# G-U-N/consolver

Measured on AMD Instinct MI355X. Metric: images/sec at 8-step ConsistencySolver 512x512 (final latents; SD1.5 UNet fp16 + PPOScheduler, CFG 3), higher is better.
Workload: dtype f16

## Files before the change

### consolver_amd/csrc/igemm.hip

```cpp
#include "ops.h"
#include <stdlib.h>
#include <type_traits>


namespace {

constexpr int BM = 128;
constexpr int BK = 64;

__device__ __attribute__((aligned(256))) unsigned g_zero_page[64];

struct IgemmParams {
    const f16* a0; const f16* a1; int c0, c1;
    int Hi, Wi, Ho, Wo, HoWo;
    int stride, upsample;
    int pad_lo;
    int M, N, KT, cpt;
    int Ktot;
    const f16* w; const f16* bias; const f16* temb; int temb_stride; const f16* res; f16* out;
    const f16* res_lo; f16* out_lo;
    const f16* a0_lo; const f16* a1_lo; int KTh;
    float* row_stats;
    const float* ln_stats; int ln_groups; float ln_inv_c, ln_eps; const float* ln_s; const float* ln_b;
    int tiles_n, nblk;
// ... 1305 lines not shown
    asm volatile("s_waitcnt vmcnt(0)" ::: "memory");
    __builtin_amdgcn_s_barrier();
    if (KT > 1) static_for<4>([&](auto nc) { piece(nc, 1, 1); });
    lds_read<0>(fw[0], SW[0][0]); lds_read<0>(fa[0][0], SA[0][0]); lds_read<2048>(fa[0][1], SA[0][0]);
    lds_read<2048>(fw[1], SW[0][0]); lds_read<2 * 2048>(fa[0][2], SA[0][0]); lds_read<3 * 2048>(fa[0][3], SA[0][0]);
    lds_read<2 * 2048>(fw[2], SW[0][0]); lds_read<3 * 2048>(fw[3], SW[0][0]);

    int kt = 0;
    auto step = [&](auto b_tag) {
        constexpr int B = decltype(b_tag)::value, BO = B ^ 1;
        static_for<NQ>([&](auto qc) {
            constexpr int q = decltype(qc)::value, ks = q / NT, i = q - ks * NT;
            if constexpr (q == QB) {
                asm volatile("s_waitcnt vmcnt(0) lgkmcnt(0)" ::: "memory");
                __builtin_amdgcn_s_barrier();
            }
            {
                constexpr int r = q + LA;
                if constexpr (r < NT) lds_read<r * 2048>(fw[r % RS], SW[B][0]);
                else if constexpr (r < NQ) lds_read<(r - NT) * 2048>(fw[r % RS], SW[B][1]);
                else lds_read<(r - NQ) * 2048>(fw[r % RS], SW[BO][0]);
            }
            if constexpr (q < MT) lds_read<q * 2048>(fa[1][q], SA[B][1]);
            if constexpr (q == QB || q == QB + 1) {
                constexpr int j0 = (q - QB) * 2;
                lds_read<j0 * 2048>(fa[0][j0], SA[BO][0]); lds_read<(j0 + 1) * 2048>(fa[0][j0 + 1], SA[BO][0]);
            }
            asm volatile("s_waitcnt lgkmcnt(%0)" :: "n"(lw_wait_count(q, NQ, LA, MT, QB)));
            __builtin_amdgcn_sched_barrier(0);
#pragma unroll
            for (int j = 0; j < MT; ++j) mfma_inplace(acc[i][j], fw[q % RS], fa[ks][j]);
            __builtin_amdgcn_sched_barrier(0);
            if constexpr (q < 5) { if (kt + 1 < KT) piece(std::integral_constant<int, 4 + q>{}, kt + 1, BO); }
            if constexpr (q >= QB) { if (kt + 2 < KT) piece(std::integral_constant<int, q - QB>{}, kt + 2, B); }
            __builtin_amdgcn_sched_barrier(0);
        });
    };
    for (;;) {
        step(std::integral_constant<int, 0>{}); if (++kt == KT) break;
        step(std::integral_constant<int, 1>{}); if (++kt == KT) break;
    }
    asm volatile("s_waitcnt vmcnt(0) lgkmcnt(0)\n s_nop 7\n s_nop 7" ::: "memory");
#pragma unroll
    for (int i = 0; i < NT; ++i)
#pragma unroll
        for (int j = 0; j < MT; ++j) asm volatile("" : "+v"(acc[i][j]));
    __builtin_amdgcn_s_barrier();
    char* const ln_tab = LNM == 1 ? lnx + BMX * 8 + wn * (2 * (BNX / 2) * 4) : lnx + wn * (BNX / 2) * 2;
    const char* const ln_rows = LNM == 1 ? lnx + wm * 64 * 8 : nullptr;
    if constexpr (GEGLU) igemm_epilogue<GEGLU, NT, MT, NT, LinearRows, 1, LNM, true>(p, acc, LinearRows{m_blk + wm * 64, p.M}, n_blk + wn * (BNX / 2), lane, smem + w * 11264, ln_tab, ln_rows);
    else igemm_epilogue<GEGLU, NT, MT, NT, LinearRows, 2, LNM, true, EPI>(p, acc, LinearRows{m_blk + wm * 64, p.M}, n_blk + wn * (BNX / 2), lane, smem + w * 11264, ln_tab, ln_rows);
}

__global__ __launch_bounds__(256) void row_stats_kernel(const f16* __restrict__ x, const f16* __restrict__ x_lo, int M, int C, float* __restrict__ stats, int lo8) {
    const int lane = threadIdx.x & 63, row = blockIdx.x * 4 + (threadIdx.x >> 6);
    if (row >= M) return;
    float s1 = 0.f, s2 = 0.f;
    for (int c = lane * 8; c < C; c += 512) {
        const f16x8 t = *reinterpret_cast<const f16x8*>(x + (size_t)row * C + c);
        float fv[8];
#pragma unroll
        for (int k = 0; k < 8; ++k) fv[k] = (float)t[k];
        if (x_lo && lo8) lo8_decode_add(fv, *reinterpret_cast<const u32x2_t*>(reinterpret_cast<const unsigned char*>(x_lo) + (size_t)row * C + c));
        else if (x_lo) {
            const f16x8 t2 = *reinterpret_cast<const f16x8*>(x_lo + (size_t)row * C + c);
#pragma unroll
            for (int k = 0; k < 8; ++k) fv[k] += (float)t2[k];
        }
#pragma unroll
        for (int k = 0; k < 8; ++k) { const float f = fv[k]; s1 += f; s2 = __builtin_fmaf(f, f, s2); }
    }
    s1 = wave_sum(s1); s2 = wave_sum(s2);
    if (lane == 0) { stats[2 * (size_t)row] = s1; stats[2 * (size_t)row + 1] = s2; }
}

__device__ __forceinline__ f16x8 splitk_reduce_item(const IgemmParams& p, const float* __restrict__ partial, int splits, int m, int n) {
    float v[8] = {0, 0, 0, 0, 0, 0, 0, 0};
    for (int s = 0; s < splits; ++s) {
        const float* src = partial + ((size_t)s * p.M + m) * p.N + n;
        const f32x4 a = *reinterpret_cast<const f32x4*>(src), b = *reinterpret_cast<const f32x4*>(src + 4);
#pragma unroll
        for (int k = 0; k < 4; ++k) { v[k] += a[k]; v[4 + k] += b[k]; }
    }
    if (p.ln_stats) {
        float s1 = 0.f, s2 = 0.f;
        const float* st = p.ln_stats + (size_t)m * p.ln_groups * 2;
        ln_row_moments(st, p.ln_groups, s1, s2);
        const float mean = s1 * p.ln_inv_c, rstd = __builtin_amdgcn_rsqf(fmaxf(__builtin_fmaf(-mean, mean, s2 * p.ln_inv_c), 0.f) + p.ln_eps), mr = mean * rstd;
#pragma unroll
        for (int k = 0; k < 8; ++k) v[k] = __builtin_fmaf(v[k], rstd, __builtin_fmaf(-mr, p.ln_s[n + k], p.ln_b[n + k]));
    } else if (p.bias) { const f16x8 t = *reinterpret_cast<const f16x8*>(p.bias + n);
#pragma unroll
        for (int k = 0; k < 8; ++k) v[k] += (float)t[k]; }
    if (p.temb) { const f16x8 t = *reinterpret_cast<const f16x8*>(p.temb + (size_t)(m / p.HoWo) * p.temb_stride + n);
#pragma unroll
        for (int k = 0; k < 8; ++k) v[k] += (float)t[k]; }
    if (p.res) { const f16x8 t = *reinterpret_cast<const f16x8*>(p.res + (size_t)m * p.N + n);
#pragma unroll
        for (int k = 0; k < 8; ++k) v[k] += (float)t[k]; }
    if (p.res && p.res_lo) {
        if (p.lo8) lo8_decode_add(v, *reinterpret_cast<const u32x2_t*>(reinterpret_cast<const unsigned char*>(p.res_lo) + (size_t)m * p.N + n));
        else { const f16x8 t = *reinterpret_cast<const f16x8*>(p.res_lo + (size_t)m * p.N + n);
#pragma unroll
            for (int k = 0; k < 8; ++k) v[k] += (float)t[k]; }
    }
    f16x8 o;
// ... 368 lines not shown
        configured = true;
    }
    hipLaunchKernelGGL(kfn, dim3(p.nblk, splits), dim3(256), lds, s, p);
    CS_CHECK_LAUNCH();
    if (splits > 1) return launch_splitk_reduce(p, (const float*)p.partial, splits, s);
    return CS_OK;
}

}

constexpr size_t LN_LDS_W8 = 256 * 8 + 2 * 2 * 160 * 4, LN_LDS_LW = 256 * 8 + 2 * 160 * 4;

static int choose_xcd_grid(int tiles_m, int tiles_n, double a_bytes, double w_bytes) {
    if (!tune().xcd_grid) return 0;
    int best = 0; double best_cost = 0.85 * (a_bytes + 8.0 * w_bytes);
    for (int pn = 2; pn <= 8; pn *= 2) {
        const int px = 8 / pn;
        if (tiles_n % pn || tiles_m % px) continue;
        const double cost = pn * a_bytes + px * w_bytes;
        if (cost < best_cost) { best_cost = cost; best = pn; }
    }
    return best;
}

double igemm_flops(const IgemmArgs& a) {
    const double M = (double)a.B * a.Ho * a.Wo;
    return 2.0 * M * a.N * (double)a.taps * (a.c0 + a.c1);
}

template <bool UP, int BN, int KH, int SCHED>
static int launch_halo_sched(const HaloParams& h, dim3 grid, size_t lds, hipStream_t s) {
    static bool configured = false;
    if (!configured) {
        constexpr size_t max_lds = 2 * (HALO_ROWS_MAX * 128) + 3 * (160 * 128);
        CS_CHECK_HIP(hipFuncSetAttribute(reinterpret_cast<const void*>(conv3_halo_kernel<UP, BN, KH, SCHED>), hipFuncAttributeMaxDynamicSharedMemorySize, (int)max_lds));
        configured = true;
    }
    hipLaunchKernelGGL((conv3_halo_kernel<UP, BN, KH, SCHED>), grid, dim3(512), lds, s, h);
    CS_CHECK_LAUNCH();
    return CS_OK;
}
template <bool UP, int BN, int KH>
static int launch_halo(const HaloParams& h, dim3 grid, size_t lds, hipStream_t s) { return launch_halo_sched<UP, BN, KH, KH == 2 ? 2 : 0>(h, grid, lds, s); }

struct LaunchInfo { bool gn_done = false; int row_groups = 0; };
static inline void route_set(int family, int tile_cols, int variant, int splits = 1) { t_igemm_route.family = family; t_igemm_route.tile_cols = tile_cols; t_igemm_route.variant = variant; t_igemm_route.splits = splits; }
static int launch_igemm_impl(const IgemmArgs& a, hipStream_t s, LaunchInfo* li) {
    const int cin = a.c0 + a.c1;
    if (!a.a0 || !a.w || !a.out) CS_FAIL(CS_E_ARG, "igemm: a0, w, out required");
    if (a.taps != 1 && a.taps != 9) CS_FAIL(CS_E_ARG, "igemm: taps must be 1 or 9");
    if (cin % BK || a.c0 % BK || (a.c1 && !a.a1)) CS_FAIL(CS_E_SHAPE, "igemm: channels (%d,%d) must be multiples of %d", a.c0, a.c1, BK);
    if (a.B <= 0 || a.Ho <= 0 || a.Wo <= 0) return (a.B < 0) ? CS_E_SHAPE : CS_OK;
    if (a.taps == 1 && (a.stride != 1 || a.upsample || a.Hi != a.Ho || a.Wi != a.Wo)) CS_FAIL(CS_E_ARG, "igemm: 1x1 needs stride 1, no upsample");
    if (a.geglu && (a.N % 256) && (a.N % 320)) CS_FAIL(CS_E_SHAPE, "igemm: GEGLU needs N %% 256 == 0 or N %% 320 == 0 (N=%d)", a.N);
    IgemmParams p;
    p.a0 = a.a0; p.a1 = a.a1; p.c0 = a.c0; p.c1 = a.c1;
    p.Hi = a.Hi; p.Wi = a.Wi; p.Ho = a.Ho; p.Wo = a.Wo; p.HoWo = a.Ho * a.Wo;
    p.stride = a.stride; p.upsample = a.upsample; p.pad_lo = a.pad_after_only ? 0 : 1;
    if (a.pad_after_only && !(a.taps == 9 && a.stride == 2)) CS_FAIL(CS_E_ARG, "igemm: pad_after_only is the stride-2 3x3 form");
    p.M = a.B * a.Ho * a.Wo; p.N = a.N; p.cpt = cin / BK; p.KT = a.taps * p.cpt; p.Ktot = a.taps * cin;
    p.w = a.w; p.bias = a.bias; p.temb = a.temb; p.temb_stride = a.temb_stride; p.res = a.res; p.out = a.out;
    p.res_lo = a.res ? a.res_lo : nullptr; p.out_lo = a.out_lo; p.lo8 = (a.lo8 && (p.res_lo || p.out_lo)) ? 1 : 0;
    const bool conv3_early = a.taps == 9;
    p.row_stats = a.row_stats;
    p.ln_stats = a.ln_stats; p.ln_groups = a.ln_groups; p.ln_inv_c = 1.0f / (float)cin; p.ln_eps = a.ln_eps; p.ln_s = a.ln_s; p.ln_b = a.ln_b;
    if (a.ln_stats) {
        if (a.taps != 1 || a.c1 || a.temb || a.res || a.out_lo || a.row_stats || a.gn_stats)
            CS_FAIL(CS_E_ARG, "igemm: a folded LayerNorm (ln_stats) is the epilogue of a plain linear layer (one source, no temb / residual / lo plane / statistics)");
        if (!a.ln_s || !a.ln_b || a.ln_groups < 1) CS_FAIL(CS_E_ARG, "igemm: ln_stats needs ln_s, ln_b and ln_groups >= 1");
    }
    if (a.row_stats && (a.geglu || a.gn_stats)) CS_FAIL(CS_E_ARG, "igemm: row_stats excludes GEGLU and gn_stats");
    if (a.row_stats && !a.row_stats_groups) CS_FAIL(CS_E_ARG, "igemm: row_stats needs row_stats_groups (the layout the chosen kernel wrote is returned there)");
    p.a0_lo = a.a0_lo; p.a1_lo = a.c1 ? a.a1_lo : nullptr; p.KTh = p.KT;
    const int lnm = a.ln_stats ? 1 : (a.row_stats && !conv3_early ? 2 : 0);
    const bool split_a = a.a0_lo != nullptr;
    if (split_a) {
        if (a.taps != 1 || a.geglu) CS_FAIL(CS_E_ARG, "igemm: a split-fp16 A operand (a0_lo) is built for 1x1 / linear layers without GEGLU");
        if (a.c1 && !a.a1_lo) CS_FAIL(CS_E_ARG, "igemm: a0_lo without a1_lo");
        p.KT = 2 * p.KTh;
    }
    if (a.geglu && a.out_lo) CS_FAIL(CS_E_ARG, "igemm: the GEGLU epilogue writes no lo plane");
    if (p.lo8 && (a.taps != 1 || a.temb || a.geglu || a.ln_stats)) CS_FAIL(CS_E_ARG, "igemm: 8-bit lo planes (lo8) are built for plain 1x1 / linear layers (the transformer hidden state)");
    p.epi_fast = tune().epi_fast;
    const int epi = (a.taps == 1 && !a.geglu && !a.ln_stats && !a.temb) ? (p.lo8 ? 1 : (p.res && p.res_lo && !p.out_lo && (p.epi_fast & 2)) ? 2 : 0) : 0;
    p.debug = tune().debug; p.partial = nullptr;
    const bool stats_ok = a.gn_stats && !a.geglu && p.HoWo % 64 == 0 && tune().gn_fuse != 0;
    p.gn_stats = stats_ok ? a.gn_stats : nullptr;
    p.gm = 1; p.pn = 0;
    const double a_bytes = 2.0 * a.B * a.Hi * a.Wi * cin, w_bytes = 2.0 * a.N * a.taps * cin;
    const int tiles_m = (p.M + BM - 1) / BM;
    int bn;
    if (a.N % 128 == 0) bn = 128;
    else if (a.N % 160 == 0) bn = 160;
    else CS_FAIL(CS_E_SHAPE, "igemm: N=%d must be a multiple of 128 or 160", a.N);
    p.tiles_n = a.N / bn; p.nblk = tiles_m * p.tiles_n;
    const bool conv3 = a.taps == 9;
    const int use_halo = tune().halo;
    const int Wo = a.upsample ? 2 * a.Wi : a.Wi, Ho = a.upsample ? 2 * a.Hi : a.Hi;
    int hbn = a.N % 160 == 0 ? 160 : (a.N % 128 == 0 ? 128 : 0);
    bool wide = false;
    const int TW = Wo >= 16 ? 16 : Wo, THmax = TW ? 256 / TW : 0, TH = Ho < THmax ? Ho : THmax;
    const bool pow2 = TW == 8 || TW == 16;
    const bool geom_ok = pow2 && TH >= 2 && (TH & (TH - 1)) == 0 && Wo % TW == 0 && Ho % TH == 0 && Ho == a.Ho && Wo == a.Wo &&
                         (!a.upsample || (TH % 2 == 0 && TW % 2 == 0 && TW / 2 + 2 >= 10));
    if (igemm_sub_pixel(a, tune())) {
        const int sbn = a.N % 160 == 0 ? 160 : 128;
        const bool f1 = a.Wi % 16 == 0 && a.Hi % 16 == 0;
        const int TWi = f1 ? 16 : 8, TRW = f1 ? 256 : 64, IPT = 256 / TRW;
        const int PX = a.Wi / TWi, PY = a.Hi / TWi, PP = PX * PY;
        const int tiles_lo = PP == 1 ? (a.B + IPT - 1) / IPT : a.B * PP, tiles_m = 4 * tiles_lo, tiles_n = a.N / sbn;
        HaloParams h;
        h.HALO_W = TWi + 2; h.HALO_IMG = (TWi + 2) * (TWi + 2); h.NHALO = IPT * h.HALO_IMG; h.NQ = (h.NHALO + 7) / 8;
        h.e = p; h.e.w = a.w_up_sub; h.e.tiles_n = tiles_n; h.e.nblk = tiles_m * tiles_n; h.e.row_stats = nullptr; h.e.pn = choose_xcd_grid(tiles_m, tiles_n, a_bytes, w_bytes * 16.0 / 9.0);
        h.x = a.a0; h.w = a.w_up_sub; h.Cin = cin; h.H = a.Hi; h.W = a.Wi; h.B = a.B; h.NC = cin / BK; h.Ho = Ho; h.Wo = Wo;
        h.tw_shift = f1 ? 4 : 3; h.trw_shift = f1 ? 8 : 6; h.PX = PX; h.PP = PP; h.splits = 1; h.partial = nullptr; h.sched = 0;
        typedef void (*lw_fn)(HaloParams);
        static const lw_fn sub[3] = {conv3_lw_kernel<false, 160, false, 1, true>, conv3_lw_kernel<false, 160, false, 2, true>, conv3_lw_kernel<false, 128, false, 1, true>};
        static bool configured_sub = false;
        if (!configured_sub) {
            for (lw_fn f : sub)
                CS_CHECK_HIP(hipFuncSetAttribute(reinterpret_cast<const void*>(f), hipFuncAttributeMaxDynamicSharedMemorySize, (int)(2 * (HALO_ROWS_MAX * 128) + 3 * (160 * 128))));
            configured_sub = true;
        }
        const size_t llw = 2 * ((size_t)h.NQ * 1024) + 3 * ((size_t)sbn * 128);
        const int sv = sbn == 128 ? 2 : f1 ? 0 : 1;
        route_set(4, sbn, sv);
        hipLaunchKernelGGL(sub[sv], dim3(h.e.nblk, 1), dim3(512), llw, s, h);
        CS_CHECK_LAUNCH();
        li->gn_done = stats_ok;
        return CS_OK;
    }
    if (use_halo && conv3 && a.stride == 1 && a.c1 == 0 && hbn && !a.geglu && geom_ok) {
        const int TRW = TH * TW, IPT = 256 / TRW;
        const int PX = Wo / TW, PY = Ho / TH, PP = PX * PY;
        const int tiles_m = PP == 1 ? (a.B + IPT - 1) / IPT : a.B * PP;
        if (a.N % 320 == 0 && tune().halo != 4 && (tiles_m * (a.N / 320) >= 192 || tune().halo == 3)) { hbn = 320; wide = true; }
        else if (a.N % 256 == 0 && tune().halo != 4 && (tiles_m * (a.N / 256) >= 192 || tune().halo == 3)) { hbn = 256; wide = true; }
        const bool lw_cin_ok = cin / BK <= LW_ZERO_CHUNKS;
        const bool lw160 = tune().conv_lw != 0 && a.N % 160 == 0 && lw_cin_ok;
        const bool lw128 = tune().conv_lw != 0 && tune().conv_lw != 3 && !lw160 && a.N % 128 == 0 && lw_cin_ok;
        const bool lw = lw160 || lw128;
        if (lw) { hbn = lw160 ? 160 : 128; wide = false; }
// ... 211 lines not shown
```

### consolver_amd/csrc/ops.h

```cpp
#pragma once
#include "common.h"

struct TuneSet {
    int halo = 1;
    int conv_lw = 1;
    int gemm_w8 = 1;
    int gemm_lw = 1;
    int gemm2_w8 = 1;
    int attn_lw = 1;
    int debug = 0;
    int gemm_gm = -1;
    int gn_fuse = 1;
    int cfg_share = 1;
    int xattn_fused = 1;
    int attn_prio = -1;
    int gemm2_prio = 0;
    int biggemm = 1;
    int attn_qt40 = 4;
    int x2_split_a = 1;
    int x2_sc_skip = 0;
    int ln_fold = 1;
    int xcd_grid = 1;
    int epi_fast = 3;
    int lo8 = 1;
    int conv_in_mfma = 1;
    int up_fold = 1;
    int head_x2 = 1;
    int conv_out_mfma = 1;
    int xattn_tile = 64;
};
extern TuneSet g_tune;
extern thread_local const TuneSet* t_tune;
inline const TuneSet& tune() { return t_tune ? *t_tune : g_tune; }
struct TuneScope {
    const TuneSet* prev;
    explicit TuneScope(const TuneSet* t) : prev(t_tune) { t_tune = t; }
    ~TuneScope() { t_tune = prev; }
    TuneScope(const TuneScope&) = delete; TuneScope& operator=(const TuneScope&) = delete;
};
int tune_apply(TuneSet& set, const char* key, int value);
TuneSet tune_snapshot();

struct IgemmArgs {
    const f16* a0; const f16* a1; int c0, c1;
    int B, Hi, Wi;
    int Ho, Wo;
    int taps;
    int stride;
    int upsample;
    int pad_after_only;
    int N;
    const f16* w;
    const f16* bias;
    const f16* temb; int temb_stride;
    const f16* res;
    f16* out;
    int geglu;
    float* splitk_ws; size_t splitk_ws_bytes;
    float* gn_stats;
// ... 177 lines not shown
```

### consolver_amd/csrc/ops_api.cpp

```cpp
#include "ops.h"
#include "../../include/consolver_hip_ops.h"
#include <cstring>

int debug_trace_read(void* dst, size_t bytes);
int debug_attn_trace_read(void* dst, size_t bytes);

#include <mutex>
TuneSet g_tune;
thread_local const TuneSet* t_tune = nullptr;
thread_local IgemmRoute t_igemm_route;
static std::mutex g_tune_write_mutex;

struct TuneKnob { const char* key; int TuneSet::* var; int lo, hi; bool pair; };
static const TuneKnob* tune_knobs(int* n) {
    static const TuneKnob k[] = {
        {"conv_halo", &TuneSet::halo, 0, 4, false},     {"gemm_lw", &TuneSet::gemm_lw, 0, 1, false},      {"gemm2_w8", &TuneSet::gemm2_w8, 0, 1, false},
        {"attn_lw", &TuneSet::attn_lw, 0, 2, false},    {"gemm_w8", &TuneSet::gemm_w8, 0, 1, false},      {"conv_lw", &TuneSet::conv_lw, 0, 3, false},
        {"gemm_big", &TuneSet::biggemm, 0, 3, false},   {"debug", &TuneSet::debug, 0, 0x7fffffff, false}, {"gemm_gm", &TuneSet::gemm_gm, -1, 64, false},
        {"gn_fuse", &TuneSet::gn_fuse, 0, 1, false},    {"xattn_fused", &TuneSet::xattn_fused, 0, 1, false}, {"cfg_share", &TuneSet::cfg_share, 0, 1, false},
        {"gemm2_prio", &TuneSet::gemm2_prio, -1, 1, false}, {"attn_prio", &TuneSet::attn_prio, -1, 1, false}, {"attn_qt40", &TuneSet::attn_qt40, 2, 4, true},
        {"x2_split_a", &TuneSet::x2_split_a, 0, 3, false}, {"x2_sc_skip", &TuneSet::x2_sc_skip, 0, 0xffff, false}, {"ln_fold", &TuneSet::ln_fold, 0, 1, false}, {"xcd_grid", &TuneSet::xcd_grid, 0, 1, false}, {"epi_fast", &TuneSet::epi_fast, 0, 3, false}, {"lo8", &TuneSet::lo8, 0, 1, false},
        {"conv_in_mfma", &TuneSet::conv_in_mfma, 0, 1, false}, {"xattn_tile", &TuneSet::xattn_tile, 64, 128, true},
        {"conv_out_mfma", &TuneSet::conv_out_mfma, 0, 1, false},
        {"up_fold", &TuneSet::up_fold, 0, 2, false},
        {"head_x2", &TuneSet::head_x2, 0, 1, false},
    };
    *n = (int)(sizeof(k) / sizeof(k[0]));
    return k;
}

int tune_apply(TuneSet& set, const char* key, int value) {
    if (!key) CS_FAIL(CS_E_ARG, "key is NULL");
    int n; const TuneKnob* k = tune_knobs(&n);
    for (int i = 0; i < n; ++i)
        if (!strcmp(key, k[i].key)) {
            const bool ok = k[i].pair ? (value == k[i].lo || value == k[i].hi) : (value >= k[i].lo && value <= k[i].hi);
            if (!ok) CS_FAIL(CS_E_ARG, "tuning key '%s': value %d outside %s%d%s%d%s", key, value, k[i].pair ? "{" : "[", k[i].lo, k[i].pair ? ", " : " .. ", k[i].hi, k[i].pair ? "}" : "]");
            set.*(k[i].var) = value;
            return CS_OK;
        }
    CS_FAIL(CS_E_ARG, "unknown tuning key '%s'", key);
}

TuneSet tune_snapshot() {
    std::lock_guard<std::mutex> lock(g_tune_write_mutex);
    return g_tune;
}

extern "C" {

int cs_set_tuning(const char* key, int value) {
    std::lock_guard<std::mutex> lock(g_tune_write_mutex);
    return tune_apply(g_tune, key, value);
}

int cs_get_tuning(const char* key, int* value) {
    if (!key || !value) CS_FAIL(CS_E_ARG, "key / value is NULL");
    int n; const TuneKnob* k = tune_knobs(&n);
    for (int i = 0; i < n; ++i)
        if (!strcmp(key, k[i].key)) { *value = tune().*(k[i].var); return CS_OK; }
    CS_FAIL(CS_E_ARG, "unknown tuning key '%s'", key);
}

int cs_reset_tuning(void) {
    std::lock_guard<std::mutex> lock(g_tune_write_mutex);
    g_tune = TuneSet();
    return CS_OK;
}

int cs_op_conv2d(const void* x0, int c0, const void* x1, int c1, int B, int Hi, int Wi, int taps, int stride, int upsample,
                 const void* w, const void* bias, int N, const void* temb, int temb_stride, const void* res, void* out,
                 void* splitk_ws, size_t splitk_ws_bytes, void* stream) {
    IgemmArgs a{};
    a.a0 = (const f16*)x0; a.a1 = (const f16*)x1; a.c0 = c0; a.c1 = c1; a.B = B; a.Hi = Hi; a.Wi = Wi;
    if (stride != 1 && stride != 2) CS_FAIL(CS_E_ARG, "conv2d: stride must be 1 or 2");
    if (stride == 2 && !upsample && ((Hi | Wi) & 1)) CS_FAIL(CS_E_SHAPE, "conv2d: stride 2 needs an even input size (got %d x %d)", Hi, Wi);
    a.Ho = upsample ? 2 * Hi : (stride == 2 ? Hi / 2 : Hi);
    a.Wo = upsample ? 2 * Wi : (stride == 2 ? Wi / 2 : Wi);
// ... 390 lines not shown
```

### consolver_amd/ops.py

```python
import collections
import ctypes as C

import torch

from . import _lib as L


def _f16(t, name):
    L.require_cuda(t, name)
    if t.dtype != torch.float16 or not t.is_contiguous():
        raise TypeError(f"{name} must be a contiguous float16 tensor")
    return t


def pack_conv_weight(w):
    co, ci = w.shape[0], w.shape[1]
    return w.reshape(co, ci, -1).permute(0, 2, 1).contiguous().to(torch.float16)


_SPLITK_WS = {}


def conv2d(x0, w_packed, bias=None, x1=None, taps=9, stride=1, upsample=False, temb=None, res=None, splitk=True, gn_stats=False, out=None, st=None):
    _f16(x0, "x0")
# ... 134 lines not shown
        if ws is None:
            ws = _SPLITK_WS[x.device] = torch.empty(64 << 20, dtype=torch.uint8, device=x.device)
    rs, G = (torch.zeros(M, N // 64, 2, dtype=torch.float32, device=x.device), C.c_int(0)) if row_stats else (None, None)
    L.check(L.lib().cs_op_linear_lo8(L.ptr(x), M, K, L.ptr(w), L.ptr(bias), N, L.ptr(res), L.ptr(res_lo8), L.ptr(out), L.ptr(out_lo),
                                     L.ptr(rs), C.byref(G) if row_stats else None,
                                     L.ptr(ws), ws.numel() if ws is not None else 0, L.stream_ptr(x.device)))
    if row_stats:
        return out, out_lo, (rs, G.value)
    return out, out_lo


def xattn_block_lo8(h, h_lo8, ln_gamma, ln_beta, wq, kv, wo, bo, heads=8, eps=1e-5, hw=None, row_stats=False):
    _f16(h, "h")
    M, Cc = h.shape
    hw = hw or M // kv.shape[0]
    out = torch.empty_like(h)
    out_lo = torch.empty(M, Cc, dtype=torch.uint8, device=h.device)
    rs = torch.zeros(M, 1, 2, dtype=torch.float32, device=h.device) if row_stats else None
    L.check(L.lib().cs_op_xattn_block_lo8(L.ptr(h), L.ptr(h_lo8), L.ptr(ln_gamma), L.ptr(ln_beta), float(eps), L.ptr(wq), L.ptr(kv), kv.shape[1],
                                          L.ptr(wo), L.ptr(bo), M, hw, Cc, heads, float((Cc // heads) ** -0.5), L.ptr(out), L.ptr(out_lo), L.ptr(rs),
                                          L.stream_ptr(h.device)))
    if row_stats:
        return out, out_lo, rs
    return out, out_lo


def row_stats_lo8(x, x_lo8):
    _f16(x, "x")
    M, Cc = x.shape
    st = torch.empty(M, 1, 2, dtype=torch.float32, device=x.device)
    L.check(L.lib().cs_op_row_stats_lo8(L.ptr(x), L.ptr(x_lo8), M, Cc, L.ptr(st), L.stream_ptr(x.device)))
    return st


def ln_dc_ratio(stats, C_in, eps=1e-5):
    M, G, _ = stats.shape
    acc = torch.zeros(1, dtype=torch.float32, device=stats.device)
    L.check(L.lib().cs_op_ln_dc_ratio(L.ptr(stats), M, G, C_in, eps, L.ptr(acc), L.stream_ptr(stats.device)))
    return float((acc / M).sqrt())


def ln_fold_pack(w, bias, gamma, beta):
    w = w.detach().to("cpu", torch.float16).contiguous()
    g = gamma.detach().to("cpu", torch.float16).contiguous()
    be = beta.detach().to("cpu", torch.float16).contiguous()
    b = bias.detach().to("cpu", torch.float16).contiguous() if bias is not None else None
    N, K = w.shape
    wo, so, bo = torch.empty_like(w), torch.empty(N, dtype=torch.float32), torch.empty(N, dtype=torch.float32)
    L.check(L.lib().cs_op_ln_fold_pack(C.c_void_p(w.data_ptr()), C.c_void_p(b.data_ptr()) if b is not None else None, C.c_void_p(g.data_ptr()),
                                       C.c_void_p(be.data_ptr()), N, K, C.c_void_p(wo.data_ptr()), C.c_void_p(so.data_ptr()), C.c_void_p(bo.data_ptr())))
    return wo, so, bo


def linear_ln(x, w_folded, ln_s, ln_b, stats, groups, eps=1e-5, geglu=False, splitk=True):
    _f16(x, "x")
    M, K = x.shape
    N = w_folded.shape[0]
    out = torch.empty(M, N // 2 if geglu else N, dtype=torch.float16, device=x.device)
    ws = None
    if splitk:
        ws = _SPLITK_WS.get(x.device)
        if ws is None:
            ws = _SPLITK_WS[x.device] = torch.empty(64 << 20, dtype=torch.uint8, device=x.device)
    L.check(L.lib().cs_op_linear_ln(L.ptr(x), M, K, L.ptr(w_folded), L.ptr(ln_s), L.ptr(ln_b), N, L.ptr(stats), int(groups), float(eps), L.ptr(out), int(geglu),
                                    L.ptr(ws), ws.numel() if ws is not None else 0, L.stream_ptr(x.device)))
    return out


def row_stats(x, x_lo=None):
    _f16(x, "x")
    M, Cc = x.shape
    st = torch.empty(M, 1, 2, dtype=torch.float32, device=x.device)
    L.check(L.lib().cs_op_row_stats(L.ptr(x), L.ptr(x_lo), M, Cc, L.ptr(st), L.stream_ptr(x.device)))
    return st


def group_norm_x2(x0, x0_lo, gamma, beta, groups=32, eps=1e-5, silu=False, x1=None, x1_lo=None):
    _f16(x0, "x0")
    B = x0.shape[0]
    c0 = x0.shape[-1]
    c1 = x1.shape[-1] if x1 is not None else 0
    HW = x0.numel() // (B * c0)
    ws = torch.empty(int(L.lib().cs_op_group_norm_workspace(B, c0 + c1)), dtype=torch.uint8, device=x0.device)
    out = torch.empty(x0.shape[:-1] + (c0 + c1,), dtype=torch.float16, device=x0.device)
    L.check(L.lib().cs_op_group_norm_x2(L.ptr(x0), L.ptr(x0_lo), c0, L.ptr(x1), L.ptr(x1_lo), c1, B, HW, groups, float(eps), int(silu),
                                        L.ptr(gamma), L.ptr(beta), L.ptr(ws), L.ptr(out), L.stream_ptr(x0.device)))
    return out


def layer_norm_x2(x, x_lo, gamma, beta, eps=1e-5):
    _f16(x, "x")
    M, Cc = x.shape
    out = torch.empty_like(x)
    L.check(L.lib().cs_op_layer_norm_x2(L.ptr(x), L.ptr(x_lo), L.ptr(gamma), L.ptr(beta), L.ptr(out), M, Cc, float(eps), L.stream_ptr(x.device)))
    return out


def xattn_block_x2(h, h_lo, ln_gamma, ln_beta, wq, kv, wo, bo, heads=8, eps=1e-5, hw=None, row_stats=False):
    _f16(h, "h")
    M, Cc = h.shape
    hw = hw or M // kv.shape[0]
    out = torch.empty_like(h)
    out_lo = torch.empty_like(h) if h_lo is not None else None
    rs = torch.zeros(M, 1, 2, dtype=torch.float32, device=h.device) if row_stats else None
    L.check(L.lib().cs_op_xattn_block_x2(L.ptr(h), L.ptr(h_lo), L.ptr(ln_gamma), L.ptr(ln_beta), float(eps), L.ptr(wq), L.ptr(kv), kv.shape[1],
                                         L.ptr(wo), L.ptr(bo), M, hw, Cc, heads, float((Cc // heads) ** -0.5), L.ptr(out), L.ptr(out_lo), L.ptr(rs),
                                         L.stream_ptr(h.device)))
    if row_stats:
        return out, out_lo, rs
    return out, out_lo

# ... 133 lines not shown
        out = torch.empty(B, HW, 64, dtype=torch.float16, device=x.device)
    L.check(L.lib().cs_op_latent_to_nhwc64(L.ptr(x), L.ptr(w), L.ptr(b), L.ptr(out), B, Cc, HW, float(in_scale), float(in_shift), L.stream_ptr(x.device)))
    return out


def pixel_linear(x, w, b, in_scale=1.0, in_shift=0.0, out=None):
    _f16(x, "x")
    B, Cc, HW = x.shape
    if out is None:
        out = torch.empty_like(x)
    L.check(L.lib().cs_op_pixel_linear(L.ptr(x), L.ptr(w), L.ptr(b), L.ptr(out), B, Cc, HW, float(in_scale), float(in_shift), L.stream_ptr(x.device)))
    return out


def pixel_affine(x, Cout, w=None, b=None, out_scale=1.0, out_shift=0.0, out=None):
    _f16(x, "x")
    B, Cin, HW = x.shape
    if out is None:
        out = torch.empty(B, Cout, HW, dtype=torch.float16, device=x.device)
    L.check(L.lib().cs_op_pixel_affine(L.ptr(x), Cin, L.ptr(w), L.ptr(b), Cout, L.ptr(out), B, HW, float(out_scale), float(out_shift), L.stream_ptr(x.device)))
    return out


def conv_down(x, w_packed, bias=None, out=None):
    _f16(x, "x")
    B, Hi, Wi, Cin = x.shape
    N = w_packed.shape[0]
    if out is None:
        out = torch.empty(B, Hi // 2, Wi // 2, N, dtype=torch.float16, device=x.device)
    L.check(L.lib().cs_op_conv_down(L.ptr(x), Cin, B, Hi, Wi, L.ptr(w_packed), L.ptr(bias), N, L.ptr(out), L.stream_ptr(x.device)))
    return out


def layer_norm(x, gamma, beta, eps=1e-5):
    _f16(x, "x")
    M, Cc = x.shape
    out = torch.empty_like(x)
    L.check(L.lib().cs_op_layer_norm(L.ptr(x), L.ptr(gamma), L.ptr(beta), L.ptr(out), M, Cc, float(eps), L.stream_ptr(x.device)))
    return out


def xattn_block(h, ln_gamma, ln_beta, wq, kv, wo, bo, heads=8, eps=1e-5, hw=None, out=None):
    _f16(h, "h")
    M, Cc = h.shape
    hw = hw or M // kv.shape[0]
    if out is None:
        out = torch.empty_like(h)
    L.check(L.lib().cs_op_xattn_block(L.ptr(h), L.ptr(ln_gamma), L.ptr(ln_beta), float(eps), L.ptr(wq), L.ptr(kv), kv.shape[1], L.ptr(wo),
                                      L.ptr(bo), M, hw, Cc, heads, float((Cc // heads) ** -0.5), L.ptr(out), L.stream_ptr(h.device)))
    return out


IgemmRoute = collections.namedtuple("IgemmRoute", "family tile_cols variant splits gn_done row_groups fallback")
IGEMM_FAMILIES = ("none", "generic", "halo", "conv3_lw", "sub_pixel", "gemm_big", "gemm_w8", "gemm_lw")


def igemm_last_route():
    v = (C.c_int * 7)()
    n = L.lib().cs_debug_igemm_last_route(v, 7)
    if n != 7:
        raise RuntimeError(f"cs_debug_igemm_last_route: {n}")
    return IgemmRoute(IGEMM_FAMILIES[v[0]], *list(v)[1:])


def set_tuning(key, value):
    L.check(L.lib().cs_set_tuning(key.encode(), int(value)))


def get_tuning(key):
    v = C.c_int(0)
    L.check(L.lib().cs_get_tuning(key.encode(), C.byref(v)))
    return v.value


def reset_tuning():
    L.check(L.lib().cs_reset_tuning())
```

Measured before the change: 74.88.

## Add A-stationary GEMM kernel for K=320 linear layers with streamed weight slices

Adds a new 512-thread kernel for 1x1/linear layers with 320 input channels. Each wave keeps its 64 rows of A in registers across the whole N range. Weight slices of 32 columns are streamed through a three-deep LDS ring using buffer_load-to-LDS, and the epilogue (bias, folded LayerNorm, GEGLU) is fused in. Half the waves are skewed to overlap epilogue stores with MFMA work. It is routed by default for large M and N>=960, replacing the tiled igemm there; the cost is heavy register use for the A fragments and hand-tuned waitcnt logic.

Result: faster. 75.68, median of 6 (+1.1%).

```diff
diff --git a/consolver_amd/csrc/igemm.hip b/consolver_amd/csrc/igemm.hip
--- a/consolver_amd/csrc/igemm.hip
+++ b/consolver_amd/csrc/igemm.hip
@@ -1381,6 +1381,225 @@
     else igemm_epilogue<GEGLU, NT, MT, NT, LinearRows, 2, LNM, true, EPI>(p, acc, LinearRows{m_blk + wm * 64, p.M}, n_blk + wn * (BNX / 2), lane, smem + w * 11264, ln_tab, ln_rows);
 }
 
+typedef unsigned u32x4_t __attribute__((ext_vector_type(4)));
+__device__ __forceinline__ void dma16_uncounted(unsigned lds_dst, unsigned voff, u32x4_t rsrc, unsigned soff) {
+    unsigned keep;
+    asm volatile("s_mov_b32 %0, m0\n\ts_mov_b32 m0, %1\n\ts_nop 4\n\tbuffer_load_dwordx4 %2, %3, %4 offen lds\n\ts_mov_b32 m0, %0"
+                 : "=&s"(keep) : "s"(lds_dst), "v"(voff), "s"(rsrc), "s"(soff) : "memory");
+}
+__device__ __forceinline__ void mfma_first(f32x4& c, const f16x8& a, const f16x8& b) {
+    asm volatile("v_mfma_f32_16x16x32_f16 %0, %1, %2, 0" : "=&v"(c) : "v"(a), "v"(b));
+}
+constexpr int AS_SLICE = 32 * 640, AS_RING = 3, AS_PATCH = 8192;
+static inline size_t gemm_as_lds(int N) { return (size_t)AS_RING * AS_SLICE + 8 * AS_PATCH + 512 * 8 + (size_t)N * 8; }
+constexpr int AS_MAX_N = (160 * 1024 - AS_RING * AS_SLICE - 8 * AS_PATCH - 512 * 8) / 8;
+
+template <bool GEGLU, int LNM>
+__global__ __launch_bounds__(512) void gemm_as_kernel(IgemmParams p) {
+    static_assert(LNM == 0 || LNM == 1, "bias or folded-LayerNorm epilogue");
+    constexpr int KS = 10, MT = 4, NQ = 2 * KS, LA = 3;
+    constexpr int G = GEGLU ? 4 : 2;
+    constexpr int CPS = GEGLU ? 16 : 32;
+    extern __shared__ __attribute__((aligned(16))) char smem[];
+    const int tid = threadIdx.x, lane = tid & 63;
+    const int w = __builtin_amdgcn_readfirstlane(tid >> 6);
+    const int m_wg = blockIdx.x * 512, m_base = m_wg + w * 64;
+    const int NS = p.N >> 5, Nout = GEGLU ? (p.N >> 1) : p.N;
+    char* const patch = smem + AS_RING * AS_SLICE + w * AS_PATCH;
+    char* const lnx = smem + AS_RING * AS_SLICE + 8 * AS_PATCH;
+    const int gq = lane >> 4, i16 = lane & 15, g4 = gq * 4;
+
+    f16x8 fa[KS][MT];
+#pragma unroll
+    for (int j = 0; j < MT; ++j) {
+        const int m = min(m_base + j * 16 + i16, p.M - 1);
+        const f16* ap = p.a0 + (size_t)m * 320 + gq * 8;
+#pragma unroll
+        for (int s = 0; s < KS; ++s) fa[s][j] = *reinterpret_cast<const f16x8*>(ap + s * 32);
+    }
+
+    const int pch = lane & 7, wr = (w & 3) * 8 + (lane >> 3);
+    const unsigned voff = (unsigned)(wr * 640 + ((pch ^ ((wr >> 1) & 7)) * 16));
+    const unsigned long long wa = (unsigned long long)(uintptr_t)p.w;
+    const u32x4_t rw = {(unsigned)wa, (unsigned)(wa >> 32) & 0xffffu, 0xffffffffu, 0x00020000u};
+    const unsigned sbase = lds_addr(smem);
+    const int kh = w >> 2;
+    auto stage = [&](int sl, int buf) __attribute__((always_inline)) {
+        const unsigned src = (unsigned)sl * AS_SLICE;
+        const unsigned dst = sbase + buf * AS_SLICE + (w & 3) * 1024;
+        dma16_uncounted(dst + kh * 4096, voff, rw, src + kh * 128);
+        dma16_uncounted(dst + (2 + kh) * 4096, voff, rw, src + (2 + kh) * 128);
+        dma16_uncounted(dst + 4 * 4096, voff, rw, src + 4 * 128);
+    };
+    stage(0, 0);
+    if (NS > 1) stage(1, 1);
+    if constexpr (LNM == 1) ln_tile_prologue(p, lnx, tid, 512, m_wg, 512, 0, p.N, 1);
+    else bias_tile_prologue(p, lnx, tid, 0, p.N);
+#pragma unroll
+    for (int s = 0; s < KS; ++s)
+#pragma unroll
+        for (int j = 0; j < MT; ++j) asm volatile("" : "+v"(fa[s][j]));
+    asm volatile("s_waitcnt vmcnt(0) lgkmcnt(0)" ::: "memory");
+    __builtin_amdgcn_s_barrier();
+
+    const int swz = (lane >> 1) & 7;
+    const unsigned wfrag0 = sbase + i16 * 128 + (gq ^ swz) * 16, wfrag1 = sbase + i16 * 128 + ((4 + gq) ^ swz) * 16;
+    f32x4 acc[2][MT];
+
+    auto top = [&](int j, int sh) __attribute__((always_inline)) {
+        const int e1 = j - 1 - sh, e2 = j - 2 - sh;
+        const bool st = (e1 >= 0 && e1 % G == G - 1) || (e2 >= 0 && e2 % G == G - 1);
+        if (j + 1 < NS) {
+            if (st) asm volatile("s_waitcnt vmcnt(11) lgkmcnt(0)" ::: "memory");
+            else asm volatile("s_waitcnt vmcnt(3) lgkmcnt(0)" ::: "memory");
+        } else {
+            if (st) asm volatile("s_waitcnt vmcnt(8) lgkmcnt(0)" ::: "memory");
+            else asm volatile("s_waitcnt vmcnt(0) lgkmcnt(0)" ::: "memory");
+        }
+        __builtin_amdgcn_s_barrier();
+        if (j + 2 < NS) {
+            int b2 = j + 2; b2 -= (b2 / AS_RING) * AS_RING;
+            stage(j + 2, b2);
+        }
+    };
+    auto mm = [&](int buf) __attribute__((always_inline)) {
+        const unsigned b0 = wfrag0 + buf * AS_SLICE, b1 = wfrag1 + buf * AS_SLICE;
+        f16x8 fw[LA + 1];
+        auto rd = [&](auto qc) __attribute__((always_inline)) {
+            constexpr int q = decltype(qc)::value, s = q >> 1, i = q & 1;
+            lds_read<(s >> 1) * 4096 + i * 2048>(fw[q % (LA + 1)], (s & 1) ? b1 : b0);
+        };
+        static_for<LA>([&](auto qc) { rd(qc); });
+        static_for<NQ>([&](auto qc) {
+            constexpr int q = decltype(qc)::value, s = q >> 1, i = q & 1;
+            if constexpr (q + LA < NQ) rd(std::integral_constant<int, (q + LA < NQ ? q + LA : 0)>{});
+            asm volatile("s_waitcnt lgkmcnt(%0)" :: "n"(NQ - 1 - q < LA ? NQ - 1 - q : LA));
+            __builtin_amdgcn_sched_barrier(0);
+#pragma unroll
+            for (int j = 0; j < MT; ++j) {
+                if constexpr (s == 0) mfma_first(acc[i][j], fw[q % (LA + 1)], fa[s][j]);
+                else mfma_inplace(acc[i][j], fw[q % (LA + 1)], fa[s][j]);
+            }
+            __builtin_amdgcn_sched_barrier(0);
+        });
+        asm volatile("s_nop 7\n s_nop 7" ::: "memory");
+#pragma unroll
+        for (int i = 0; i < 2; ++i)
+#pragma unroll
+            for (int j = 0; j < MT; ++j) asm volatile("" : "+v"(acc[i][j]));
+    };
+    auto epi = [&](int j) __attribute__((always_inline)) {
+        const int slot = j % G;
+        const float* const tabf = reinterpret_cast<const float*>(lnx + 512 * 8);
+        const f16* const tabh = reinterpret_cast<const f16*>(lnx);
+#pragma unroll
+        for (int i = 0; i < (GEGLU ? 1 : 2); ++i) {
+            const int n = j * 32 + i * 16 + g4;
+            float bv[4] = {0.f, 0.f, 0.f, 0.f}, bg[4] = {0.f, 0.f, 0.f, 0.f};
+            float sv[4] = {0.f, 0.f, 0.f, 0.f}, sg[4] = {0.f, 0.f, 0.f, 0.f};
+            auto tables = [&](int zo) __attribute__((always_inline)) {
+                if constexpr (LNM == 1) {
+                    const f32x4 t = *reinterpret_cast<const f32x4*>(tabf + zo + n), u = *reinterpret_cast<const f32x4*>(tabf + zo + p.N + n);
+#pragma unroll
+                    for (int r = 0; r < 4; ++r) { bv[r] = t[r]; sv[r] = u[r]; }
+                    if constexpr (GEGLU) {
+                        const f32x4 t2 = *reinterpret_cast<const f32x4*>(tabf + zo + n + 16), u2 = *reinterpret_cast<const f32x4*>(tabf + zo + p.N + n + 16);
+#pragma unroll
+                        for (int r = 0; r < 4; ++r) { bg[r] = t2[r]; sg[r] = u2[r]; }
+                    }
+                } else if (p.bias) {
+                    const f16x4 t = *reinterpret_cast<const f16x4*>(tabh + zo + n);
+#pragma unroll
+                    for (int r = 0; r < 4; ++r) bv[r] = (float)t[r];
+                    if constexpr (GEGLU) {
+                        const f16x4 u = *reinterpret_cast<const f16x4*>(tabh + zo + n + 16);
+#pragma unroll
+                        for (int r = 0; r < 4; ++r) bg[r] = (float)u[r];
+                    }
+                }
+            };
+            if constexpr (!GEGLU) tables(0);
+#pragma unroll
+            for (int jm = 0; jm < MT; ++jm) {
+                int zo = 0;
+                asm volatile("" : "+v"(zo));
+                if constexpr (GEGLU) tables(zo);
+                float ln_r = 0.f, ln_mr = 0.f;
+                if constexpr (LNM == 1) {
+                    const f32x2 t = *reinterpret_cast<const f32x2*>(lnx + zo + (w * 64 + jm * 16 + i16) * 8);
+                    ln_r = t[0]; ln_mr = t[1];
+                }
+                f32x4 val;
+                if constexpr (LNM == 1) {
+#pragma unroll
+                    for (int r = 0; r < 4; ++r) val[r] = __builtin_fmaf(acc[i][jm][r], ln_r, __builtin_fmaf(-ln_mr, sv[r], bv[r]));
+                } else {
+#pragma unroll
+                    for (int r = 0; r < 4; ++r) val[r] = acc[i][jm][r] + bv[r];
+                }
+                f16x4 o;
+                if constexpr (GEGLU) {
+                    const f32x4 ga = acc[1][jm];
+                    f32x4 gt;
+                    if constexpr (LNM == 1) {
+#pragma unroll
+                        for (int r = 0; r < 4; ++r) gt[r] = __builtin_fmaf(ga[r], ln_r, __builtin_fmaf(-ln_mr, sg[r], bg[r]));
+                    } else {
+#pragma unroll
+                        for (int r = 0; r < 4; ++r) gt[r] = ga[r] + bg[r];
+                    }
+                    f32x2 g01, g23;
+                    gelu_erf4(f32x2{gt[0], gt[1]}, f32x2{gt[2], gt[3]}, g01, g23);
+                    o[0] = (f16)(val[0] * g01[0]); o[1] = (f16)(val[1] * g01[1]);
+                    o[2] = (f16)(val[2] * g23[0]); o[3] = (f16)(val[3] * g23[1]);
+                } else {
+#pragma unroll
+                    for (int r = 0; r < 4; ++r) o[r] = (f16)val[r];
+                }
+                const int row = jm * 16 + i16, col = slot * CPS + (GEGLU ? 0 : i * 16) + g4;
+                *reinterpret_cast<f16x4*>(patch + row * 128 + (((col >> 3) ^ (row & 7)) << 4) + (col & 7) * 2) = o;
+                if constexpr (GEGLU) __builtin_amdgcn_sched_barrier(0);
+            }
+        }
+        const int colbase = (j / G) * 64, ch = lane & 7, r8 = lane >> 3;
+        if (slot == G - 1) {
+#pragma unroll
+            for (int k = 0; k < 8; ++k) {
+                const int row = r8 + 8 * k;
+                const f16x8 v = *reinterpret_cast<const f16x8*>(patch + row * 128 + ((ch ^ r8) << 4));
+                const int m = min(m_base + row, p.M - 1);
+                *reinterpret_cast<f16x8*>(p.out + (size_t)m * Nout + colbase + ch * 8) = v;
+            }
+        } else if (j == NS - 1) {
+            const int chn = (slot + 1) * CPS / 8;
+#pragma unroll
+            for (int k = 0; k < 8; ++k) {
+                const int row = r8 + 8 * k;
+                const f16x8 v = *reinterpret_cast<const f16x8*>(patch + row * 128 + ((ch ^ r8) << 4));
+                const int m = min(m_base + row, p.M - 1);
+                if (ch < chn) *reinterpret_cast<f16x8*>(p.out + (size_t)m * Nout + colbase + ch * 8) = v;
+            }
+        }
+    };
+
+    if (w < 4) {
+        for (int j = 0, buf = 0; j < NS; ++j) {
+            top(j, 0);
+            mm(buf);
+            epi(j);
+            buf = buf == AS_RING - 1 ? 0 : buf + 1;
+        }
+    } else {
+        for (int j = 0, buf = 0; j <= NS; ++j) {
+            if (j < NS) top(j, 1);
+            if (j > 0) epi(j - 1);
+            if (j == NS) break;
+            mm(buf);
+            buf = buf == AS_RING - 1 ? 0 : buf + 1;
+        }
+    }
+}
+
 __global__ __launch_bounds__(256) void row_stats_kernel(const f16* __restrict__ x, const f16* __restrict__ x_lo, int M, int C, float* __restrict__ stats, int lo8) {
     const int lane = threadIdx.x & 63, row = blockIdx.x * 4 + (threadIdx.x >> 6);
     if (row >= M) return;
@@ -1855,7 +2074,11 @@
     if (cin % BK || a.c0 % BK || (a.c1 && !a.a1)) CS_FAIL(CS_E_SHAPE, "igemm: channels (%d,%d) must be multiples of %d", a.c0, a.c1, BK);
     if (a.B <= 0 || a.Ho <= 0 || a.Wo <= 0) return (a.B < 0) ? CS_E_SHAPE : CS_OK;
     if (a.taps == 1 && (a.stride != 1 || a.upsample || a.Hi != a.Ho || a.Wi != a.Wo)) CS_FAIL(CS_E_ARG, "igemm: 1x1 needs stride 1, no upsample");
-    if (a.geglu && (a.N % 256) && (a.N % 320)) CS_FAIL(CS_E_SHAPE, "igemm: GEGLU needs N %% 256 == 0 or N %% 320 == 0 (N=%d)", a.N);
+    const long long as_m = (long long)a.B * a.Ho * a.Wo;
+    const bool as_route = tune().gemm_as != 0 && a.taps == 1 && a.c1 == 0 && cin == 320 && !a.a0_lo && !a.temb && !a.res && !a.out_lo && !a.row_stats && !a.gn_stats &&
+                          a.N > 0 && a.N % 32 == 0 && a.N <= AS_MAX_N && !tune().debug && (double)as_m * 640 < 4.0e9 &&
+                          (tune().gemm_as == 2 || ((as_m + 511) / 512 >= 192 && a.N >= 960));
+    if (!as_route && a.geglu && (a.N % 256) && (a.N % 320)) CS_FAIL(CS_E_SHAPE, "igemm: GEGLU needs N %% 256 == 0 or N %% 320 == 0 (N=%d)", a.N);
     IgemmParams p;
     p.a0 = a.a0; p.a1 = a.a1; p.c0 = a.c0; p.c1 = a.c1;
     p.Hi = a.Hi; p.Wi = a.Wi; p.Ho = a.Ho; p.Wo = a.Wo; p.HoWo = a.Ho * a.Wo;
@@ -1891,6 +2114,20 @@
     p.gn_stats = stats_ok ? a.gn_stats : nullptr;
     p.gm = 1; p.pn = 0;
     const double a_bytes = 2.0 * a.B * a.Hi * a.Wi * cin, w_bytes = 2.0 * a.N * a.taps * cin;
+    if (as_route) {
+        typedef void (*as_fn)(IgemmParams);
+        static const as_fn asv[4] = {gemm_as_kernel<false, 0>, gemm_as_kernel<true, 0>, gemm_as_kernel<false, 1>, gemm_as_kernel<true, 1>};
+        static bool configured_as = false;
+        if (!configured_as) {
+            for (as_fn f : asv) CS_CHECK_HIP(hipFuncSetAttribute(reinterpret_cast<const void*>(f), hipFuncAttributeMaxDynamicSharedMemorySize, (int)gemm_as_lds(AS_MAX_N)));
+            configured_as = true;
+        }
+        const int av = 2 * lnm + (a.geglu ? 1 : 0);
+        route_set(8, 32, av);
+        hipLaunchKernelGGL(asv[av], dim3((p.M + 511) / 512), dim3(512), gemm_as_lds(a.N), s, p);
+        CS_CHECK_LAUNCH();
+        return CS_OK;
+    }
     const int tiles_m = (p.M + BM - 1) / BM;
     int bn;
     if (a.N % 128 == 0) bn = 128;
diff --git a/consolver_amd/csrc/ops.h b/consolver_amd/csrc/ops.h
--- a/consolver_amd/csrc/ops.h
+++ b/consolver_amd/csrc/ops.h
@@ -5,6 +5,7 @@
     int halo = 1;
     int conv_lw = 1;
     int gemm_w8 = 1;
+    int gemm_as = 1;
     int gemm_lw = 1;
     int gemm2_w8 = 1;
     int attn_lw = 1;
diff --git a/consolver_amd/csrc/ops_api.cpp b/consolver_amd/csrc/ops_api.cpp
--- a/consolver_amd/csrc/ops_api.cpp
+++ b/consolver_amd/csrc/ops_api.cpp
@@ -24,6 +24,7 @@
         {"conv_out_mfma", &TuneSet::conv_out_mfma, 0, 1, false},
         {"up_fold", &TuneSet::up_fold, 0, 2, false},
         {"head_x2", &TuneSet::head_x2, 0, 1, false},
+        {"gemm_as", &TuneSet::gemm_as, 0, 2, false},
     };
     *n = (int)(sizeof(k) / sizeof(k[0]));
     return k;
diff --git a/consolver_amd/ops.py b/consolver_amd/ops.py
--- a/consolver_amd/ops.py
+++ b/consolver_amd/ops.py
@@ -210,11 +210,12 @@
     return wo, so, bo
 
 
-def linear_ln(x, w_folded, ln_s, ln_b, stats, groups, eps=1e-5, geglu=False, splitk=True):
+def linear_ln(x, w_folded, ln_s, ln_b, stats, groups, eps=1e-5, geglu=False, splitk=True, out=None):
     _f16(x, "x")
     M, K = x.shape
     N = w_folded.shape[0]
-    out = torch.empty(M, N // 2 if geglu else N, dtype=torch.float16, device=x.device)
+    if out is None:
+        out = torch.empty(M, N // 2 if geglu else N, dtype=torch.float16, device=x.device)
     ws = None
     if splitk:
         ws = _SPLITK_WS.get(x.device)
@@ -454,7 +455,7 @@
 
 
 IgemmRoute = collections.namedtuple("IgemmRoute", "family tile_cols variant splits gn_done row_groups fallback")
-IGEMM_FAMILIES = ("none", "generic", "halo", "conv3_lw", "sub_pixel", "gemm_big", "gemm_w8", "gemm_lw")
+IGEMM_FAMILIES = ("none", "generic", "halo", "conv3_lw", "sub_pixel", "gemm_big", "gemm_w8", "gemm_lw", "gemm_as")
 
 
 def igemm_last_route():
```
